# FlyCole/Dream2Real

Measured on AMD Instinct MI355X. Metric: candidate renders scored/sec (640x360), higher is better.
Workload: dtype bf16 + fp16 NeRF MLP operands (fp32 accumulate; the library's default: the reference's tiny-cuda-nn operand type, same MFMA rate; --opt mlp_f16=0 = bf16 operands)

## Files before the change

### dream2real_amd/csrc/clip.hip

```cpp
#include "d2r_internal.h"

#include <type_traits>

#include <math.h>
#include <stdio.h>
#include <stdlib.h>

#include <algorithm>
#include <deque>
#include <mutex>

typedef __bf16 bf16x8 __attribute__((ext_vector_type(8)));
typedef float f32x16 __attribute__((ext_vector_type(16)));
typedef float f32x4 __attribute__((ext_vector_type(4)));

struct ClipWeights {
    const uint16_t *w_patch;
    const float *cls, *pos;
    const float *pre_w, *pre_b;
    struct Layer {
        const float *ln1_w, *ln1_b, *ln2_w, *ln2_b;
        const uint16_t *w_qkv, *w_o, *w_fc1, *w_fc2;
        const float *b_qkv, *b_o, *b_fc1, *b_fc2;
        const uint16_t *wf_qkv = nullptr, *wf_fc1 = nullptr;
// ... 203 lines not shown
                           uint16_t *__restrict__ patches, uint32_t Kp_pad)
{
    size_t i = (size_t)blockIdx.x * blockDim.x + threadIdx.x;
    size_t total = (size_t)n * 3 * S * S;
    if (i >= total) return;
    uint32_t x = i % S, y = (i / S) % S, c = (i / ((size_t)S * S)) % 3, img = i / ((size_t)3 * S * S);
    uint32_t g = S / P;
    size_t rowi = (size_t)img * g * g + (y / P) * g + (x / P);
    patches[rowi * Kp_pad + (c * P + (y % P)) * P + (x % P)] = f2bf(pv[i]);
}


__device__ __forceinline__ size_t lo8_off(uint32_t M_pad, size_t row, uint32_t col)
{
    return ((((size_t)(col >> 6) * (M_pad >> 6)) + (row >> 6)) << 12) + ((row & 31) << 7) + (((col & 63) >> 3) << 4) + (((row >> 5) & 1) << 3) + (col & 7);
}
__device__ __forceinline__ float split8_value(uint32_t hi16, int32_t lo8) { return __uint_as_float((hi16 << 16) + (uint32_t)(lo8 << 8)); }
__device__ __forceinline__ int32_t split8_round(float x, uint32_t hi_bits )
{
    const int32_t dlt = (int32_t)__float_as_uint(x) - (int32_t)hi_bits;
    return min(dlt + 0x80, 0x7fff);
}

enum { EPI_F32 = 0, EPI_BIAS_BF16 = 1, EPI_BIAS_GELU_BF16 = 2, EPI_BIAS_RESID_F32 = 3,
       EPI_LN_BIAS_BF16 = 4, EPI_LN_BIAS_GELU_BF16 = 5, EPI_RESID_STATS_F32X = 6, EPI_RESID_STATS_BF16 = 7,
       EPI_RESID_STATS_SPLIT = 8, EPI_RESID_STATS_SPLIT8 = 9,
       EPI_F8_BIAS_BF16 = 10, EPI_F8_BIAS_GELU_Q8 = 11, EPI_F8_RESID_STATS_SPLIT8 = 12, EPI_KINDS = 13 };
#define EPI_IS_F8(E) ((E) >= EPI_F8_BIAS_BF16)
#define EPI_IS_LN(E) ((E) == EPI_LN_BIAS_BF16 || (E) == EPI_LN_BIAS_GELU_BF16)
#define EPI_IS_STATS(E) ((E) == EPI_RESID_STATS_F32X || (E) == EPI_RESID_STATS_BF16 || (E) == EPI_RESID_STATS_SPLIT || (E) == EPI_RESID_STATS_SPLIT8 || (E) == EPI_F8_RESID_STATS_SPLIT8)
#define EPI_IS_F32_LAYOUT(E) ((E) == EPI_F32 || (E) == EPI_BIAS_RESID_F32)

struct EpiAux {
    const float *cs;
    const float2 *ab;
    uint16_t *xb;
    float2 *part;
    uint16_t *xlo;
    uint32_t hm_rows;
    uint32_t a_rs, a_ks;
    const uint32_t *m_dev;
    const uint32_t *a_scale;
    float w_scale;
    uint8_t *q8;
    uint8_t *q8_scale;
};

__device__ __forceinline__ uint32_t q8_scale_byte(float amax)
{
    const int e = (int)((__float_as_uint(amax) + 0x200000u) >> 23);
    return (uint32_t)min(max(e - 8, 1), 253);
}
__device__ __forceinline__ float q8_inv_scale(uint32_t byte) { return __uint_as_float((254u - byte) << 23); }
__device__ __forceinline__ size_t q8_scale_off(uint32_t M_pad, size_t row, uint32_t group)
{
    return ((((size_t)(group >> 1) * (M_pad >> 6) + (row >> 6)) * 32 + (row & 31)) << 2) + (((row >> 5) & 1) << 1) + (group & 1u);
}
typedef float f32x2 __attribute__((ext_vector_type(2)));
__device__ __forceinline__ uint2 q8_pack8(const float (&f)[8], float inv)
{
    const f32x2 i2 = f32x2{inv, inv};
    const f32x2 q0 = f32x2{f[0], f[1]} * i2, q1 = f32x2{f[2], f[3]} * i2, q2 = f32x2{f[4], f[5]} * i2, q3 = f32x2{f[6], f[7]} * i2;
    uint32_t a = __builtin_amdgcn_cvt_pk_fp8_f32(q0[0], q0[1], 0, false);
    a = __builtin_amdgcn_cvt_pk_fp8_f32(q1[0], q1[1], a, true);
    uint32_t b = __builtin_amdgcn_cvt_pk_fp8_f32(q2[0], q2[1], 0, false);
    b = __builtin_amdgcn_cvt_pk_fp8_f32(q3[0], q3[1], b, true);
    return make_uint2(a, b);
}

#ifdef D2R_DEV
#include "clip_dev.h"
#else
#define D2R_GEMM_ABLATE 0
#define D2R_ATTN_ABLATE 0
#define D2R_F8_EXP 0
#define D2R_F8_VAR 0
#define STAMP(var)
#endif
#ifndef D2R_GEMM_LATE_DRAIN
#define D2R_GEMM_LATE_DRAIN 1
#endif
#ifndef D2R_GEMM_MFMA16
#define D2R_GEMM_MFMA16 1
#endif
#ifndef D2R_GEMM_PRIO
#define D2R_GEMM_PRIO 2
#endif
#define BM 256
#define BK 64
#define GEMM_THREADS 512

__device__ __forceinline__ uint32_t lds_off(uint32_t row, uint32_t chunk)
{
    return row * 128u + ((chunk ^ ((row >> 1) & 7u)) << 4);
}

__device__ __forceinline__ void glds16(const void *g, uint32_t lds_byte_addr)
{
    asm volatile("s_mov_b32 m0, %1\n\ts_nop 0\n\tglobal_load_lds_dwordx4 %0, off" : : "v"(g), "s"(lds_byte_addr) : "memory");
}
__device__ __forceinline__ uint32_t lds_addr(const void *p)
{
    return (uint32_t)(size_t)(__attribute__((address_space(3))) const void *)p;
}
template <int N>
__device__ __forceinline__ void wait_vmcnt()
{
    static_assert(N >= 0 && N < 64, "vmcnt is a 6-bit field");
    asm volatile("s_waitcnt vmcnt(%0)" ::"n"(N) : "memory");
}

#define EP_LD 68u
#define EP_WAVE_FLOATS (8u * EP_LD)
struct NoHook { __device__ __forceinline__ void operator()() const {} };
__device__ __forceinline__ float row16_sum(float x)
{
    x += __int_as_float(__builtin_amdgcn_update_dpp(0, __float_as_int(x), 0x128, 0xf, 0xf, false));
    x += __int_as_float(__builtin_amdgcn_update_dpp(0, __float_as_int(x), 0x124, 0xf, 0xf, false));
    x += __int_as_float(__builtin_amdgcn_update_dpp(0, __float_as_int(x), 0x122, 0xf, 0xf, false));
    x += __int_as_float(__builtin_amdgcn_update_dpp(0, __float_as_int(x), 0x121, 0xf, 0xf, false));
    return x;
}
__device__ __forceinline__ float row8_sum(float x)
{
    x += __int_as_float(__builtin_amdgcn_update_dpp(0, __float_as_int(x), 0xB1, 0xf, 0xf, false));
    x += __int_as_float(__builtin_amdgcn_update_dpp(0, __float_as_int(x), 0x4E, 0xf, 0xf, false));
    x += __int_as_float(__builtin_amdgcn_update_dpp(0, __float_as_int(x), 0x141, 0xf, 0xf, false));
    return x;
}
__device__ __forceinline__ float row8_max(float x)
{
    x = fmaxf(x, __int_as_float(__builtin_amdgcn_update_dpp(0, __float_as_int(x), 0xB1, 0xf, 0xf, false)));
    x = fmaxf(x, __int_as_float(__builtin_amdgcn_update_dpp(0, __float_as_int(x), 0x4E, 0xf, 0xf, false)));
    x = fmaxf(x, __int_as_float(__builtin_amdgcn_update_dpp(0, __float_as_int(x), 0x141, 0xf, 0xf, false)));
    return x;
}
__device__ __forceinline__ float bf_lo(uint32_t u) { return __uint_as_float(u << 16); }
__device__ __forceinline__ float bf_hi(uint32_t u) { return __uint_as_float(u & 0xffff0000u); }

template <int EPI, int MT, typename Hook = NoHook>
__device__ __forceinline__ void gemm_epilogue(f32x16 (&acc)[MT][2], float *ep, uint32_t lane,
                                              uint32_t row0, uint32_t col0, const float *__restrict__ bias,
                                              void *__restrict__ Cout, uint32_t N, const EpiAux &aux,
                                              const float2 *ab_lds, Hook hook = Hook())
{
    const uint32_t ep_addr = __builtin_amdgcn_readfirstlane(lds_addr(ep));
    auto transpose_in = [&](int i, int p8) {
        if (D2R_GEMM_ABLATE & 256) return;
        asm volatile("s_mov_b32 m0, %8\n\ts_nop 0\n\t"
                     "ds_write_addtid_b32 %0 offset:0\n\tds_write_addtid_b32 %1 offset:272\n\t"
                     "ds_write_addtid_b32 %2 offset:544\n\tds_write_addtid_b32 %3 offset:816\n\t"
                     "ds_write_addtid_b32 %4 offset:1088\n\tds_write_addtid_b32 %5 offset:1360\n\t"
                     "ds_write_addtid_b32 %6 offset:1632\n\tds_write_addtid_b32 %7 offset:1904"
                     :
                     : "v"(acc[i][0][4 * p8 + 0]), "v"(acc[i][0][4 * p8 + 1]), "v"(acc[i][0][4 * p8 + 2]), "v"(acc[i][0][4 * p8 + 3]),
                       "v"(acc[i][1][4 * p8 + 0]), "v"(acc[i][1][4 * p8 + 1]), "v"(acc[i][1][4 * p8 + 2]), "v"(acc[i][1][4 * p8 + 3]),
                       "s"(ep_addr)
                     : "memory");
    };
    static_assert(EP_LD == 68u, "the ds_write_addtid offsets above are (4 j + r) * EP_LD * 4 bytes");
    auto ep_at = [](uint32_t R, uint32_t c) -> uint32_t { return ((c >> 5) * 4u + (R & 3u)) * EP_LD + (R >> 2) * 32u + (c & 31u); };
    if (EPI_IS_F32_LAYOUT(EPI)) {
        const uint32_t c4 = (lane & 15) * 4, rl0 = lane >> 4;
        const uint32_t col = col0 + c4;
        constexpr bool RESID_F32 = EPI == EPI_BIAS_RESID_F32;
        float4 bv = make_float4(0.f, 0.f, 0.f, 0.f);
// ... 1461 lines not shown
            }
        }
    }
}

template <bool CAUSAL>
__global__ __launch_bounds__(ATTN_THREADS, 4) void k_attention(const uint16_t *__restrict__ QKV, uint16_t *__restrict__ AO, uint32_t T,
                                                              uint32_t T_pad, uint32_t d, uint32_t M_pad)
{
    constexpr uint32_t TH = ATTN_THREADS;
    extern __shared__ __attribute__((aligned(16))) uint8_t smem[];
    uint8_t *Ks = smem;
    uint16_t *Vt = (uint16_t *)(smem + (size_t)T_pad * 128);
    const uint32_t vstride = T_pad + 4;
    const uint32_t head = blockIdx.x, img = blockIdx.y;
    const uint32_t tid = threadIdx.x, lane = tid & 63, wave = tid >> 6, li = lane & 31, hi = lane >> 5;
    const size_t row_base = (size_t)img * T;
    const uint32_t ld = 64, H = d >> 6;
    const uint16_t *Qg = QKV + ((size_t)head * M_pad + row_base) * 64;
    const uint16_t *Kg = QKV + ((size_t)(H + head) * M_pad + row_base) * 64;
    const uint16_t *Vg = QKV + ((size_t)(2 * H + head) * M_pad + row_base) * 64;

    const uint32_t n_qt = (T + 31) / 32, n_kt = T_pad / 32;
    uint4 qf[4];
    {
        const uint32_t qrow0 = wave * 32 + li;
#pragma unroll
        for (int s = 0; s < 4; s++)
            qf[s] = qrow0 < T ? *(const uint4 *)(Qg + (size_t)qrow0 * ld + 16 * s + 8 * hi) : make_uint4(0, 0, 0, 0);
    }
    {
        const uint32_t ks0 = __builtin_amdgcn_readfirstlane(lds_addr(Ks));
        for (uint32_t b = __builtin_amdgcn_readfirstlane(wave); b < T_pad / 8; b += TH / 64) {
            const uint32_t row = b * 8 + (lane >> 3), src_row = row < T ? row : T - 1;
            glds16(Kg + (size_t)src_row * ld + ((lane & 7) ^ ((row >> 1) & 7u)) * 8, ks0 + b * 1024);
        }
    }
    for (uint32_t i = tid; i < (T_pad / 4) * 8; i += TH) {
        const uint32_t kb = (i >> 3) * 4, c = i & 7;
        uint4 v[4];
#pragma unroll
        for (int k = 0; k < 4; k++)
            v[k] = *(const uint4 *)(Vg + (size_t)(kb + k < T ? kb + k : T - 1) * ld + c * 8);
        const uint32_t *w0 = (const uint32_t *)&v[0], *w1 = (const uint32_t *)&v[1];
        const uint32_t *w2 = (const uint32_t *)&v[2], *w3 = (const uint32_t *)&v[3];
#pragma unroll
        for (int p = 0; p < 4; p++) {
            uint2 lo, hi2;
            lo.x = __builtin_amdgcn_perm(w1[p], w0[p], 0x05040100);
            lo.y = __builtin_amdgcn_perm(w3[p], w2[p], 0x05040100);
            hi2.x = __builtin_amdgcn_perm(w1[p], w0[p], 0x07060302);
            hi2.y = __builtin_amdgcn_perm(w3[p], w2[p], 0x07060302);
            *(uint2 *)(Vt + (size_t)(c * 8 + 2 * p) * vstride + kb) = lo;
            *(uint2 *)(Vt + (size_t)(c * 8 + 2 * p + 1) * vstride + kb) = hi2;
        }
    }
    wait_vmcnt<0>();
    __syncthreads();
    for (uint32_t qt = wave; qt < n_qt; qt += TH / 64) {
        if (qt != wave) {
            const uint32_t qrow = qt * 32 + li;
#pragma unroll
            for (int s = 0; s < 4; s++)
                qf[s] = qrow < T ? *(const uint4 *)(Qg + (size_t)qrow * ld + 16 * s + 8 * hi) : make_uint4(0, 0, 0, 0);
        }
        attn_qtile<CAUSAL>(Ks, Vt, vstride, qf, qt, T, n_kt, li, hi, AO, row_base, M_pad, head);
    }
}

#define ATTN_Q_SCALE (0.125f * 1.4426950408889634f)
#define ATS_THREADS 512
#define ATS_STAGES 5
#define ATS_SLOT 8192u
#define ATS_DEFER 8.0f
typedef short s16x4 __attribute__((ext_vector_type(4)));
typedef __attribute__((address_space(3))) const uint8_t *lds_cptr;
__device__ __forceinline__ uint2 lds_read_tr16(lds_cptr p)
{
    union { s16x4 s; uint2 u; } c;
    c.s = __builtin_amdgcn_ds_read_tr16_b64_v4i16((__attribute__((address_space(3))) s16x4 *)p);
    return c.u;
}

template <int NR>
__device__ __forceinline__ void ats_softmax(f32x16 &sacc, f32x16 &o0, f32x16 &o1, float &m_run, float &l_run, uint4 (&pb)[2])
{
#if D2R_ATTN_ABLATE & 32
    l_run += sacc[0];
    o0[0] += sacc[1];
#else
    float tmax;
    if constexpr (NR == 16) {
        float a, b;
        asm("v_max3_f32 %0, %1, %2, %3" : "=v"(a) : "v"(sacc[0]), "v"(sacc[1]), "v"(sacc[2]));
        asm("v_max3_f32 %0, %1, %2, %3" : "=v"(b) : "v"(sacc[3]), "v"(sacc[4]), "v"(sacc[5]));
        asm("v_max3_f32 %0, %1, %2, %0" : "+v"(a) : "v"(sacc[6]), "v"(sacc[7]));
        asm("v_max3_f32 %0, %1, %2, %0" : "+v"(b) : "v"(sacc[8]), "v"(sacc[9]));
        asm("v_max3_f32 %0, %1, %2, %0" : "+v"(a) : "v"(sacc[10]), "v"(sacc[11]));
        asm("v_max3_f32 %0, %1, %2, %0" : "+v"(b) : "v"(sacc[12]), "v"(sacc[13]));
        asm("v_max3_f32 %0, %1, %2, %0" : "+v"(a) : "v"(sacc[14]), "v"(sacc[15]));
        asm("v_max_f32 %0, %1, %2" : "=v"(tmax) : "v"(a), "v"(b));
    } else {
        float a;
        asm("v_max3_f32 %0, %1, %2, %3" : "=v"(a) : "v"(sacc[0]), "v"(sacc[1]), "v"(sacc[2]));
        asm("v_max_f32 %0, %1, %2" : "=v"(tmax) : "v"(a), "v"(sacc[3]));
    }
    {
        typedef unsigned u32x2 __attribute__((ext_vector_type(2)));
        const u32x2 r = __builtin_amdgcn_permlane32_swap(__float_as_uint(tmax), __float_as_uint(tmax), false, false);
        asm("v_max_f32 %0, %1, %2" : "=v"(tmax) : "v"(r[0]), "v"(r[1]));
    }
    if (__builtin_amdgcn_ballot_w64(tmax > ATS_DEFER) != 0) {
        const float dm = fmaxf(tmax, 0.f);
        const float alpha = __builtin_amdgcn_exp2f(-dm);
        l_run *= alpha;
#pragma unroll
        for (int r = 0; r < 16; r++) {
            o0[r] *= alpha;
            o1[r] *= alpha;
        }
#pragma unroll
        for (int r = 0; r < NR; r++) sacc[r] -= dm;
        m_run += dm;
    }
    if constexpr (NR == 16) {
        typedef float f32x2 __attribute__((ext_vector_type(2)));
        f32x2 pr[8];
#pragma unroll
        for (int q = 0; q < 8; q++) {
            pr[q] = f32x2{__builtin_amdgcn_exp2f(sacc[2 * q]), __builtin_amdgcn_exp2f(sacc[2 * q + 1])};
            asm volatile("" : "+v"(pr[q]));
            sacc[2 * q] = pr[q].x;
            sacc[2 * q + 1] = pr[q].y;
        }
        const f32x2 a0 = pr[0] + pr[4], a1 = pr[1] + pr[5], a2 = pr[2] + pr[6], a3 = pr[3] + pr[7];
        const f32x2 b0 = a0 + a2, b1 = a1 + a3;
        const f32x2 s2 = b0 + b1;
        l_run += s2.x + s2.y;
    } else {
#pragma unroll
        for (int r = 0; r < 4; r++) sacc[r] = __builtin_amdgcn_exp2f(sacc[r]);
        l_run += (sacc[0] + sacc[1]) + (sacc[2] + sacc[3]);
    }
#endif
    pb[0].x = pack2(sacc[0], sacc[1]);
    pb[0].y = pack2(sacc[2], sacc[3]);
    if constexpr (NR == 16) {
        pb[0].z = pack2(sacc[4], sacc[5]);
        pb[0].w = pack2(sacc[6], sacc[7]);
        pb[1] = make_uint4(pack2(sacc[8], sacc[9]), pack2(sacc[10], sacc[11]), pack2(sacc[12], sacc[13]), pack2(sacc[14], sacc[15]));
    } else {
        pb[0].z = pb[0].w = 0u;
        pb[1] = make_uint4(0u, 0u, 0u, 0u);
    }
}

template <int NW, bool Q8 = false>
__global__ __launch_bounds__(NW * 64, NW == 8 ? 4 : 1) void k_attention_s(const uint16_t *__restrict__ QKV, uint16_t *__restrict__ AO, uint32_t T,
                                                                          uint32_t d, uint32_t M_pad, uint32_t qt0, uint8_t *__restrict__ AOS = nullptr)
{
    extern __shared__ __attribute__((aligned(16))) uint8_t smem[];
    constexpr int NS = 8 / NW;
    const uint32_t head = blockIdx.x, img = blockIdx.y;
    const uint32_t tid = threadIdx.x, lane = tid & 63, wave = __builtin_amdgcn_readfirstlane(tid >> 6), li = lane & 31, hi = lane >> 5;
    const size_t row_base = (size_t)img * T;
    const uint32_t H = d >> 6;
// ... 115 lines not shown
        for (int s = 0; s < ((D2R_ATTN_ABLATE & 64) ? 0 : 2); s++) {
            if (s == 1 && short_tile) break;
            union { uint4 u; bf16x8 v; } p, va0, va1;
            p.u = pb[s];
            const uint2 a00 = lds_read_tr16(v0 + 2048u * s), a01 = lds_read_tr16(v0 + 2048u * s + 1024u);
            const uint2 a10 = lds_read_tr16(v1 + 2048u * s), a11 = lds_read_tr16(v1 + 2048u * s + 1024u);
            va0.u = make_uint4(a00.x, a00.y, a01.x, a01.y);
            va1.u = make_uint4(a10.x, a10.y, a11.x, a11.y);
            o0 = __builtin_amdgcn_mfma_f32_32x32x16_bf16(va0.v, p.v, o0, 0, 0, 0);
            o1 = __builtin_amdgcn_mfma_f32_32x32x16_bf16(va1.v, p.v, o1, 0, 0, 0);
        }
        if constexpr (!LAST) {
#pragma unroll
            for (int r = 0; r < 16; r++) sacc[r] = (D2R_ATTN_ABLATE & 128) ? __uint_as_float(ka[r & 3].x) : 0.f;
            if (!(D2R_ATTN_ABLATE & 128)) {
                typedef float f32x2 __attribute__((ext_vector_type(2)));
                f32x2 nm = {-m_run, -m_run}, pr[8];
#pragma unroll
                for (int q = 0; q < 8; q++) asm volatile("v_mov_b64 %0, %1" : "=v"(pr[q]) : "v"(nm));
#pragma unroll
                for (int q = 0; q < 8; q++) {
                    sacc[2 * q] = pr[q].x;
                    sacc[2 * q + 1] = pr[q].y;
                }
            }
#pragma unroll
            for (int s = 0; s < ((D2R_ATTN_ABLATE & 128) ? 0 : 4); s++) s_mfma(sacc, s);
        }
    };
    using std::integral_constant;
    const integral_constant<bool, false> no{};
    const integral_constant<bool, true> yes{};
    uint32_t kt = 0;
    for (; kt + ATS_STAGES - 1 < n_kt; kt++) tile(kt, integral_constant<int, ATS_STAGES - 3>{}, yes, no);
    if (n_kt - kt == 4) { tile(kt, integral_constant<int, 2>{}, no, no); kt++; }
    if (n_kt - kt == 3) { tile(kt, integral_constant<int, 1>{}, no, no); kt++; }
    if (n_kt - kt == 2) { tile(kt, integral_constant<int, 0>{}, no, no); kt++; }
    tile(kt, integral_constant<int, 0>{}, no, yes);
    wait_vmcnt<0>();
    if (!active) return;
    const float inv_l = 1.0f / half_sum(l_run);
    typedef unsigned u32x2 __attribute__((ext_vector_type(2)));
    const uint32_t lane_e = __builtin_amdgcn_mbcnt_hi(~0u, __builtin_amdgcn_mbcnt_lo(~0u, 0u));
    const uint32_t qrow_e = qt * 32 + (lane_e & 31);
    if constexpr (Q8) {
        float am = 0.f;
#pragma unroll
        for (int r = 0; r < 16; r++) am = fmaxf(am, fmaxf(fabsf(o0[r]), fabsf(o1[r])));
        am *= inv_l;
        const u32x2 ams = __builtin_amdgcn_permlane32_swap(__float_as_uint(am), __float_as_uint(am), false, false);
        const uint32_t sb = q8_scale_byte(fmaxf(__uint_as_float(ams[0]), __uint_as_float(ams[1])));
        const float sc = inv_l * q8_inv_scale(sb);
        uint8_t *dst8 = (uint8_t *)AO + (((size_t)head * M_pad + row_base + qrow_e) << 6) + 8 * (lane_e >> 5);
#pragma unroll
        for (int t = 0; t < 2; t++) {
            const f32x16 &o = t ? o1 : o0;
#pragma unroll
            for (int g = 0; g < 2; g++) {
                uint32_t a = __builtin_amdgcn_cvt_pk_fp8_f32(o[8 * g + 0] * sc, o[8 * g + 1] * sc, 0, false);
                a = __builtin_amdgcn_cvt_pk_fp8_f32(o[8 * g + 2] * sc, o[8 * g + 3] * sc, a, true);
                uint32_t b = __builtin_amdgcn_cvt_pk_fp8_f32(o[8 * g + 4] * sc, o[8 * g + 5] * sc, 0, false);
                b = __builtin_amdgcn_cvt_pk_fp8_f32(o[8 * g + 6] * sc, o[8 * g + 7] * sc, b, true);
                const u32x2 x = __builtin_amdgcn_permlane32_swap(a, b, false, false);
                if (qrow_e < T) *(uint2 *)(dst8 + 32 * t + 16 * g) = make_uint2(x[0], x[1]);
            }
        }
        if (qrow_e < T && lane_e < 32) AOS[q8_scale_off(M_pad, row_base + qrow_e, head)] = (uint8_t)sb;
        return;
    }
    uint16_t *dst = AO + ((size_t)head * M_pad + row_base + qrow_e) * 64 + 8 * (lane_e >> 5);
#pragma unroll
    for (int t = 0; t < 2; t++) {
        const f32x16 &o = t ? o1 : o0;
#pragma unroll
        for (int g = 0; g < 2; g++) {
            uint32_t a0 = pack2(o[8 * g + 0] * inv_l, o[8 * g + 1] * inv_l), a1 = pack2(o[8 * g + 2] * inv_l, o[8 * g + 3] * inv_l);
            uint32_t b0 = pack2(o[8 * g + 4] * inv_l, o[8 * g + 5] * inv_l), b1 = pack2(o[8 * g + 6] * inv_l, o[8 * g + 7] * inv_l);
            const u32x2 x = __builtin_amdgcn_permlane32_swap(a0, b0, false, false);
            const u32x2 y = __builtin_amdgcn_permlane32_swap(a1, b1, false, false);
            if (qrow_e < T) *(uint4 *)(dst + 32 * t + 16 * g) = make_uint4(x[0], y[0], x[1], y[1]);
        }
    }
}

__global__ __launch_bounds__(256) void k_attention_cls(const uint16_t *__restrict__ QKV, const uint16_t *__restrict__ Q_cls,
                                                       uint16_t *__restrict__ AO_cls, uint32_t T, uint32_t d, uint32_t M_pad,
                                                       uint32_t n_heads, uint32_t n_items)
{
    __shared__ float ps[4][1024];
    const uint32_t lane = threadIdx.x & 63, w = threadIdx.x >> 6;
    const uint32_t item = blockIdx.x * 4 + w;
    if (item >= n_items) return;
    const uint32_t img = item / n_heads, head = item - img * n_heads, H = d >> 6;
    const size_t row0 = (size_t)img * T;
    const uint16_t *Qg = Q_cls ? Q_cls + (size_t)img * d + head * 64 : QKV + ((size_t)head * M_pad + row0) * 64;
    const uint16_t *Kg = QKV + ((size_t)(H + head) * M_pad + row0) * 64;
    const uint16_t *Vg = QKV + ((size_t)(2 * H + head) * M_pad + row0) * 64;
    float q[64];
    {
        const uint4 *qp = (const uint4 *)Qg;
#pragma unroll
        for (int c = 0; c < 8; c++) {
            const uint4 v = qp[c];
            q[8 * c + 0] = bf_lo(v.x); q[8 * c + 1] = bf_hi(v.x); q[8 * c + 2] = bf_lo(v.y); q[8 * c + 3] = bf_hi(v.y);
            q[8 * c + 4] = bf_lo(v.z); q[8 * c + 5] = bf_hi(v.z); q[8 * c + 6] = bf_lo(v.w); q[8 * c + 7] = bf_hi(v.w);
        }
    }
    float mx = -INFINITY;
    for (uint32_t key = lane; key < T; key += 64) {
        const uint4 *kp = (const uint4 *)(Kg + (size_t)key * 64);
        float a = 0.f;
#pragma unroll
        for (int c = 0; c < 8; c++) {
            const uint4 v = kp[c];
            a = fmaf(q[8 * c + 0], bf_lo(v.x), a); a = fmaf(q[8 * c + 1], bf_hi(v.x), a);
            a = fmaf(q[8 * c + 2], bf_lo(v.y), a); a = fmaf(q[8 * c + 3], bf_hi(v.y), a);
            a = fmaf(q[8 * c + 4], bf_lo(v.z), a); a = fmaf(q[8 * c + 5], bf_hi(v.z), a);
            a = fmaf(q[8 * c + 6], bf_lo(v.w), a); a = fmaf(q[8 * c + 7], bf_hi(v.w), a);
        }
        ps[w][key] = a;
        mx = fmaxf(mx, a);
    }
#pragma unroll
    for (int o = 32; o > 0; o >>= 1) mx = fmaxf(mx, __shfl_xor(mx, o));
    float sum = 0.f;
    for (uint32_t key = lane; key < T; key += 64) {
        const float p = __builtin_amdgcn_exp2f(ps[w][key] - mx);
        ps[w][key] = p;
        sum += p;
    }
    sum = wave_sum(sum);
    __builtin_amdgcn_wave_barrier();
    float o = 0.f;
    for (uint32_t key = 0; key < T; key++) o = fmaf(ps[w][key], __uint_as_float((uint32_t)Vg[(size_t)key * 64 + lane] << 16), o);
    AO_cls[(size_t)img * d + head * 64 + lane] = f2bf(o / sum);
}

__global__ void k_gather_cls(const float *__restrict__ X, const uint16_t *__restrict__ Xhi, const uint16_t *__restrict__ Xlo,
                             uint32_t M_pad, uint32_t T, uint32_t d, uint32_t n, float *__restrict__ X_cls, int lo8 = 0)
{
    const uint32_t i = blockIdx.x * blockDim.x + threadIdx.x;
    if (i >= n * d) return;
    const uint32_t img = i / d, c = i - img * d;
    const size_t row = (size_t)img * T;
    float v;
    if (Xhi) {
        const size_t xo = ((size_t)(c >> 6) * M_pad + row) * 64 + (c & 63);
        v = __uint_as_float((uint32_t)Xhi[xo] << 16);
        if (Xlo && lo8) v = split8_value(Xhi[xo], ((const int8_t *)Xlo)[lo8_off(M_pad, row, c)]);
        else if (Xlo) v += __uint_as_float((uint32_t)Xlo[xo] << 16);
    } else {
        v = X[row * d + c];
    }
    X_cls[i] = v;
}

__global__ void k_gather_cls_operand(const uint16_t *__restrict__ Xhi, const float2 *__restrict__ AB, uint32_t M_pad, uint32_t T,
                                     uint32_t d, uint32_t n, uint16_t *__restrict__ Xq, float2 *__restrict__ ABq)
{
    const uint32_t i = blockIdx.x * blockDim.x + threadIdx.x, per = d / 8;
    if (i >= n * per) return;
    const uint32_t img = i / per, c = (i - img * per) * 8;
    const size_t row = (size_t)img * T;
    *(uint4 *)(Xq + (size_t)img * d + c) = *(const uint4 *)(Xhi + ((size_t)(c >> 6) * M_pad + row) * 64 + (c & 63));
    if (c == 0) ABq[img] = AB[row];
}
// ... 1081 lines not shown
```

Measured before the change: 28620.

## Rewrite CLIP attention kernel around 16x16x32 MFMA tiles with per-half-tile query handling

Adds a new default variant of the streaming attention kernel that uses 16x16x32 bf16 MFMA instead of the 32x32x16 form. Each 32-row query tile is split into two 16-row halves so a tile with only one live half skips that half's work, and the softmax reductions are rebuilt around permlane swaps for the new accumulator layout. The last key tile is masked at 16-key granularity so half-empty tails skip a V read and MFMA. It adds a second large code path, and the old ablation masks now only build with the legacy form.

After: 28620. Within noise of the previous version (-0.0%).

```diff
diff --git a/dream2real_amd/csrc/clip.hip b/dream2real_amd/csrc/clip.hip
--- a/dream2real_amd/csrc/clip.hip
+++ b/dream2real_amd/csrc/clip.hip
@@ -309,6 +309,12 @@
 #endif
 #ifndef D2R_GEMM_MFMA16
 #define D2R_GEMM_MFMA16 1
+#endif
+#ifndef D2R_ATTN_MFMA16
+#define D2R_ATTN_MFMA16 1
+#endif
+#if D2R_ATTN_MFMA16 && D2R_ATTN_ABLATE
+#error "the D2R_ATTN_ABLATE masks are wired into the 32x32x16 form of k_attention_s only: build them with -DD2R_ATTN_MFMA16=0"
 #endif
 #ifndef D2R_GEMM_PRIO
 #define D2R_GEMM_PRIO 2
@@ -1936,6 +1942,7 @@
     return c.u;
 }
 
+#if !D2R_ATTN_MFMA16
 template <int NR>
 __device__ __forceinline__ void ats_softmax(f32x16 &sacc, f32x16 &o0, f32x16 &o1, float &m_run, float &l_run, uint4 (&pb)[2])
 {
@@ -2217,6 +2224,331 @@
         }
     }
 }
+#else
+template <int NQ>
+__device__ __forceinline__ float ats_qmax(float (&t)[2])
+{
+    typedef unsigned u32x2 __attribute__((ext_vector_type(2)));
+    float x;
+    u32x2 r = __builtin_amdgcn_permlane32_swap(__float_as_uint(t[0]), __float_as_uint(t[NQ - 1]), false, false);
+    asm("v_max_f32 %0, %1, %2" : "=v"(x) : "v"(r[0]), "v"(r[1]));
+    r = __builtin_amdgcn_permlane16_swap(__float_as_uint(x), __float_as_uint(x), false, false);
+    asm("v_max_f32 %0, %1, %2" : "=v"(x) : "v"(r[0]), "v"(r[1]));
+    if constexpr (NQ == 2) {
+        r = __builtin_amdgcn_permlane32_swap(__float_as_uint(x), __float_as_uint(x), false, false);
+        t[0] = __uint_as_float(r[0]);
+        t[1] = __uint_as_float(r[1]);
+    } else {
+        t[0] = x;
+    }
+    return x;
+}
+template <int NQ>
+__device__ __forceinline__ void ats_qsum(float (&t)[2])
+{
+    typedef unsigned u32x2 __attribute__((ext_vector_type(2)));
+    u32x2 r = __builtin_amdgcn_permlane32_swap(__float_as_uint(t[0]), __float_as_uint(t[NQ - 1]), false, false);
+    float x = __uint_as_float(r[0]) + __uint_as_float(r[1]);
+    r = __builtin_amdgcn_permlane16_swap(__float_as_uint(x), __float_as_uint(x), false, false);
+    x = __uint_as_float(r[0]) + __uint_as_float(r[1]);
+    if constexpr (NQ == 2) {
+        r = __builtin_amdgcn_permlane32_swap(__float_as_uint(x), __float_as_uint(x), false, false);
+        t[0] = __uint_as_float(r[0]);
+        t[1] = __uint_as_float(r[1]);
+    } else {
+        t[0] = x;
+    }
+}
+
+typedef float f32x2 __attribute__((ext_vector_type(2)));
+typedef unsigned ats_u32x4 __attribute__((ext_vector_type(4)));
+template <int NK, int NQ>
+__device__ __forceinline__ void ats_softmax(f32x4 (&s)[2][2], f32x4 (&o)[4][2], f32x2 (&nm_run)[2], f32x2 (&l_run)[2], ats_u32x4 (&pb)[2])
+{
+    float t[2];
+#pragma unroll
+    for (int qb = 0; qb < NQ; qb++) {
+        float a;
+        asm("v_max3_f32 %0, %1, %2, %3" : "=v"(a) : "v"(s[0][qb][0]), "v"(s[0][qb][1]), "v"(s[0][qb][2]));
+        if constexpr (NK == 2) {
+            asm("v_max3_f32 %0, %1, %2, %0" : "+v"(a) : "v"(s[0][qb][3]), "v"(s[1][qb][0]));
+            asm("v_max3_f32 %0, %1, %2, %0" : "+v"(a) : "v"(s[1][qb][1]), "v"(s[1][qb][2]));
+            asm("v_max_f32 %0, %1, %2" : "=v"(t[qb]) : "v"(a), "v"(s[1][qb][3]));
+        } else {
+            asm("v_max_f32 %0, %1, %2" : "=v"(t[qb]) : "v"(a), "v"(s[0][qb][3]));
+        }
+    }
+    const float vote = ats_qmax<NQ>(t);
+    if (__builtin_amdgcn_ballot_w64(vote > ATS_DEFER) != 0) {
+#pragma unroll
+        for (int qb = 0; qb < NQ; qb++) {
+            const float dm = fmaxf(t[qb], 0.f);
+            const float alpha = __builtin_amdgcn_exp2f(-dm);
+            l_run[qb] *= alpha;
+#pragma unroll
+            for (int db = 0; db < 4; db++) o[db][qb] *= alpha;
+#pragma unroll
+            for (int kb = 0; kb < NK; kb++) s[kb][qb] -= dm;
+            nm_run[qb] -= dm;
+        }
+    }
+#pragma unroll
+    for (int qb = 0; qb < NQ; qb++) {
+        f32x2 pr[2 * NK];
+#pragma unroll
+        for (int kb = 0; kb < NK; kb++)
+#pragma unroll
+            for (int h = 0; h < 2; h++) {
+                f32x2 &p = pr[2 * kb + h];
+                p = f32x2{__builtin_amdgcn_exp2f(s[kb][qb][2 * h]), __builtin_amdgcn_exp2f(s[kb][qb][2 * h + 1])};
+                asm volatile("" : "+v"(p));
+                s[kb][qb][2 * h] = p.x;
+                s[kb][qb][2 * h + 1] = p.y;
+            }
+        auto pk_add = [](f32x2 a, f32x2 b) {
+            f32x2 r;
+            asm("v_pk_add_f32 %0, %1, %2" : "=v"(r) : "v"(a), "v"(b));
+            return r;
+        };
+        if constexpr (NK == 2) l_run[qb] = pk_add(l_run[qb], pk_add(pk_add(pr[0], pr[2]), pk_add(pr[1], pr[3])));
+        else l_run[qb] = pk_add(l_run[qb], pk_add(pr[0], pr[1]));
+        pb[qb][0] = pack2(s[0][qb][0], s[0][qb][1]);
+        pb[qb][1] = pack2(s[0][qb][2], s[0][qb][3]);
+        if constexpr (NK == 2) {
+            pb[qb][2] = pack2(s[1][qb][0], s[1][qb][1]);
+            pb[qb][3] = pack2(s[1][qb][2], s[1][qb][3]);
+        } else {
+            pb[qb][2] = pb[qb][3] = 0u;
+        }
+    }
+}
+
+template <int NW, bool Q8 = false>
+__global__ __launch_bounds__(NW * 64, NW == 8 ? 4 : 1) void k_attention_s(const uint16_t *__restrict__ QKV, uint16_t *__restrict__ AO, uint32_t T,
+                                                                          uint32_t d, uint32_t M_pad, uint32_t qt0, uint8_t *__restrict__ AOS = nullptr)
+{
+    extern __shared__ __attribute__((aligned(16))) uint8_t smem[];
+    constexpr int NS = 8 / NW;
+    const uint32_t head = blockIdx.x, img = blockIdx.y;
+    const uint32_t tid = threadIdx.x, lane = tid & 63, wave = __builtin_amdgcn_readfirstlane(tid >> 6), l16 = lane & 15, g = lane >> 4;
+    const size_t row_base = (size_t)img * T;
+    const uint32_t H = d >> 6;
+    const uint32_t n_kt = (T + 31) / 32;
+    const uint32_t qt = qt0 + blockIdx.z * NW + wave;
+    const bool active = __builtin_amdgcn_readfirstlane(qt < n_kt ? 1u : 0u) != 0u;
+    const bool one_qb = __builtin_amdgcn_readfirstlane(qt * 32 + 16 >= T ? 1u : 0u) != 0u;
+    const uint16_t *Qg = QKV + ((size_t)head * M_pad + row_base) * 64;
+    const uint16_t *src_k = QKV + ((size_t)(H + head) * M_pad + row_base) * 64, *src_v = QKV + ((size_t)(2 * H + head) * M_pad + row_base) * 64;
+    const uint32_t smem0 = __builtin_amdgcn_readfirstlane(lds_addr(smem));
+    uint32_t slot_req = 0, slot_k = 0, slot_v = 0;
+    auto advance = [](uint32_t &slot) { slot = slot + ATS_SLOT == ATS_STAGES * ATS_SLOT ? 0u : slot + ATS_SLOT; };
+    uint32_t src_off[NS], dst_off[NS], r_loc[NS];
+    bool is_v[NS];
+#pragma unroll
+    for (int j = 0; j < NS; j++) {
+        const uint32_t c = wave + (uint32_t)j * NW;
+        is_v[j] = c >= 4;
+        r_loc[j] = (c & 3) * 8 + (is_v[j] ? (lane >> 1) & 7u : lane >> 3);
+        src_off[j] = (is_v[j] ? 2 * (lane >> 4) + (lane & 1) : (lane & 7) ^ ((r_loc[j] >> 1) & 7u)) * 8;
+        dst_off[j] = (is_v[j] ? 4096u : 0u) + (c & 3) * 1024u;
+    }
+    auto request = [&](uint32_t kt) {
+#pragma unroll
+        for (int j = 0; j < NS; j++) {
+            const uint32_t row = kt * 32 + r_loc[j];
+            glds16((is_v[j] ? src_v : src_k) + (size_t)(row < T ? row : T - 1) * 64 + src_off[j], smem0 + slot_req + dst_off[j]);
+        }
+        advance(slot_req);
+    };
+    ats_u32x4 qv[4];
+    {
+        const uint32_t qrow = qt * 32 + l16;
+        const uint32_t qr0 = active && qrow < T ? qrow : T - 1, qr1 = active && qrow + 16 < T ? qrow + 16 : T - 1;
+        const uint16_t *qp0 = Qg + (size_t)qr0 * 64 + 8 * g, *qp1 = Qg + (size_t)qr1 * 64 + 8 * g;
+        asm volatile("global_load_dwordx4 %0, %4, off\n\tglobal_load_dwordx4 %1, %4, off offset:64\n\t"
+                     "global_load_dwordx4 %2, %5, off\n\tglobal_load_dwordx4 %3, %5, off offset:64"
+                     : "=&v"(qv[0]), "=&v"(qv[1]), "=&v"(qv[2]), "=&v"(qv[3]) : "v"(qp0), "v"(qp1) : "memory");
+    }
+    static_assert(ATS_STAGES == 5, "the waits below are written for a five-slot ring");
+#pragma unroll
+    for (uint32_t c = 0; c < ATS_STAGES - 1; c++) request(c);
+    asm volatile("s_waitcnt vmcnt(%4)" : "+v"(qv[0]), "+v"(qv[1]), "+v"(qv[2]), "+v"(qv[3]) : "n"(4 * NS) : "memory");
+    wait_vmcnt<3 * NS>();
+    __syncthreads();
+
+    uint32_t koff[2];
+#pragma unroll
+    for (int kk = 0; kk < 2; kk++) koff[kk] = lds_off(l16, 4 * kk + g);
+    const uint32_t vrow = 4 * g + (l16 >> 2);
+    const uint32_t voff = 4096u + (vrow >> 3) * 1024u + (vrow & 7u) * 32u + (l16 & 3u) * 8u;
+    const uint32_t n_last = T - (n_kt - 1) * 32;
+
+    f32x4 o[4][2], s[2][2];
+    f32x2 nm_run[2] = {f32x2{0.f, 0.f}, f32x2{0.f, 0.f}};
+    f32x2 l_run[2] = {f32x2{0.f, 0.f}, f32x2{0.f, 0.f}};
+    ats_u32x4 ka[2][2];
+    auto read_k = [&]() {
+#pragma unroll
+        for (int kb = 0; kb < 2; kb++)
+#pragma unroll
+            for (int kk = 0; kk < 2; kk++) ka[kb][kk] = *(const __attribute__((address_space(3))) ats_u32x4 *)((lds_cptr)(size_t)(smem0 + slot_k + koff[kk]) + 2048u * kb);
+        advance(slot_k);
+    };
+    auto mfma = [](ats_u32x4 a, ats_u32x4 b, f32x4 &acc) {
+        acc = __builtin_amdgcn_mfma_f32_16x16x32_bf16(__builtin_bit_cast(bf16x8, a), __builtin_bit_cast(bf16x8, b), acc, 0, 0, 0);
+    };
+    using std::integral_constant;
+    const integral_constant<bool, false> no{};
+    const integral_constant<bool, true> yes{};
+    auto run = [&](auto nq_tag) {
+        constexpr int NQ = decltype(nq_tag)::value;
+        auto s_mfma = [&]() {
+#pragma unroll
+            for (int kk = 0; kk < 2; kk++)
+#pragma unroll
+                for (int kb = 0; kb < 2; kb++)
+#pragma unroll
+                    for (int qb = 0; qb < NQ; qb++) mfma(ka[kb][kk], qv[2 * qb + kk], s[kb][qb]);
+        };
+#pragma unroll
+        for (int db = 0; db < 4; db++)
+#pragma unroll
+            for (int qb = 0; qb < 2; qb++) o[db][qb] = f32x4{0.f, 0.f, 0.f, 0.f};
+        read_k();
+        if (active) {
+#pragma unroll
+            for (int kb = 0; kb < 2; kb++)
+#pragma unroll
+                for (int qb = 0; qb < 2; qb++) s[kb][qb] = f32x4{0.f, 0.f, 0.f, 0.f};
+            s_mfma();
+            float t[2] = {0.f, 0.f};
+#pragma unroll
+            for (int qb = 0; qb < NQ; qb++) {
+                t[qb] = s[0][qb][0];
+#pragma unroll
+                for (int r = 1; r < 8; r++) t[qb] = fmaxf(t[qb], s[r >> 2][qb][r & 3]);
+            }
+            ats_qmax<NQ>(t);
+#pragma unroll
+            for (int qb = 0; qb < NQ; qb++) {
+                nm_run[qb] = f32x2{-t[qb], -t[qb]};
+#pragma unroll
+                for (int kb = 0; kb < 2; kb++) s[kb][qb] -= t[qb];
+            }
+        }
+        auto tile = [&](uint32_t kt, auto wait_tag, auto req_tag, auto last_tag) {
+            constexpr int WAIT = decltype(wait_tag)::value;
+            constexpr bool LAST = decltype(last_tag)::value, REQ = decltype(req_tag)::value;
+            if constexpr (!LAST) {
+                wait_vmcnt<WAIT * NS>();
+                __syncthreads();
+                if constexpr (REQ) request(kt + ATS_STAGES - 1);
+                read_k();
+            }
+            const lds_cptr vp = (lds_cptr)(size_t)(smem0 + slot_v + voff);
+            advance(slot_v);
+            if (!active) return;
+            ats_u32x4 pb[2];
+            auto pv = [&](auto full_tag) {
+#pragma unroll
+                for (int db = 0; db < 4; db++) {
+                    const uint2 a0 = lds_read_tr16(vp + 256u * db);
+                    const uint2 a1 = decltype(full_tag)::value ? lds_read_tr16(vp + 256u * db + 2048u) : make_uint2(0u, 0u);
+#pragma unroll
+                    for (int qb = 0; qb < NQ; qb++) mfma(ats_u32x4{a0.x, a0.y, a1.x, a1.y}, pb[qb], o[db][qb]);
+                }
+            };
+            if (LAST && n_last <= 16) {
+#pragma unroll
+                for (int qb = 0; qb < NQ; qb++)
+#pragma unroll
+                    for (int r = 0; r < 4; r++) s[0][qb][r] = 4 * g + (uint32_t)r < n_last ? s[0][qb][r] : -INFINITY;
+                ats_softmax<1, NQ>(s, o, nm_run, l_run, pb);
+                pv(no);
+            } else {
+                if (LAST && n_last < 32) {
+#pragma unroll
+                    for (int qb = 0; qb < NQ; qb++)
+#pragma unroll
+                        for (int r = 0; r < 4; r++) s[1][qb][r] = 16 + 4 * g + (uint32_t)r < n_last ? s[1][qb][r] : -INFINITY;
+                }
+                ats_softmax<2, NQ>(s, o, nm_run, l_run, pb);
+                pv(yes);
+            }
+            if constexpr (!LAST) {
+#pragma unroll
+                for (int qb = 0; qb < NQ; qb++) {
+                    const f32x2 nm = nm_run[qb];
+#pragma unroll
+                    for (int kb = 0; kb < 2; kb++) {
+                        f32x2 lo, hi;
+                        asm volatile("v_mov_b64 %0, %1" : "=v"(lo) : "v"(nm));
+                        asm volatile("v_mov_b64 %0, %1" : "=v"(hi) : "v"(nm));
+                        s[kb][qb] = f32x4{lo.x, lo.y, hi.x, hi.y};
+                    }
+                }
+                s_mfma();
+            }
+        };
+        uint32_t kt = 0;
+        for (; kt + ATS_STAGES - 1 < n_kt; kt++) tile(kt, integral_constant<int, ATS_STAGES - 3>{}, yes, no);
+        if (n_kt - kt == 4) { tile(kt, integral_constant<int, 2>{}, no, no); kt++; }
+        if (n_kt - kt == 3) { tile(kt, integral_constant<int, 1>{}, no, no); kt++; }
+        if (n_kt - kt == 2) { tile(kt, integral_constant<int, 0>{}, no, no); kt++; }
+        tile(kt, integral_constant<int, 0>{}, no, yes);
+        wait_vmcnt<0>();
+        if (!active) return;
+        float inv_l[2];
+#pragma unroll
+        for (int qb = 0; qb < 2; qb++) inv_l[qb] = l_run[qb].x + l_run[qb].y;
+        ats_qsum<NQ>(inv_l);
+#pragma unroll
+        for (int qb = 0; qb < NQ; qb++) inv_l[qb] = 1.0f / inv_l[qb];
+        typedef unsigned u32x2 __attribute__((ext_vector_type(2)));
+        const uint32_t lane_e = __builtin_amdgcn_mbcnt_hi(~0u, __builtin_amdgcn_mbcnt_lo(~0u, 0u));
+        const uint32_t ge = lane_e >> 4, dim_e = 16 * (ge & 1) + 8 * (ge >> 1);
+#pragma unroll
+        for (int qb = 0; qb < NQ; qb++) {
+            const uint32_t qrow_e = qt * 32 + 16 * qb + (lane_e & 15);
+            if constexpr (Q8) {
+                float am[2] = {0.f, 0.f};
+#pragma unroll
+                for (int db = 0; db < 4; db++)
+#pragma unroll
+                    for (int r = 0; r < 4; r++) am[0] = fmaxf(am[0], fabsf(o[db][qb][r]));
+                am[0] *= inv_l[qb];
+                ats_qmax<1>(am);
+                const uint32_t sb = q8_scale_byte(am[0]);
+                const float sc = inv_l[qb] * q8_inv_scale(sb);
+                uint8_t *dst8 = (uint8_t *)AO + (((size_t)head * M_pad + row_base + qrow_e) << 6) + dim_e;
+#pragma unroll
+                for (int dp = 0; dp < 2; dp++) {
+                    const f32x4 &oa = o[2 * dp][qb], &ob = o[2 * dp + 1][qb];
+                    uint32_t a = __builtin_amdgcn_cvt_pk_fp8_f32(oa[0] * sc, oa[1] * sc, 0, false);
+                    a = __builtin_amdgcn_cvt_pk_fp8_f32(oa[2] * sc, oa[3] * sc, a, true);
+                    uint32_t b = __builtin_amdgcn_cvt_pk_fp8_f32(ob[0] * sc, ob[1] * sc, 0, false);
+                    b = __builtin_amdgcn_cvt_pk_fp8_f32(ob[2] * sc, ob[3] * sc, b, true);
+                    const u32x2 x = __builtin_amdgcn_permlane16_swap(a, b, false, false);
+                    if (qrow_e < T) *(uint2 *)(dst8 + 32 * dp) = make_uint2(x[0], x[1]);
+                }
+                if (qrow_e < T && lane_e < 16) AOS[q8_scale_off(M_pad, row_base + qrow_e, head)] = (uint8_t)sb;
+            } else {
+                uint16_t *dst = AO + ((size_t)head * M_pad + row_base + qrow_e) * 64 + dim_e;
+                const float il = inv_l[qb];
+#pragma unroll
+                for (int dp = 0; dp < 2; dp++) {
+                    const f32x4 &oa = o[2 * dp][qb], &ob = o[2 * dp + 1][qb];
+                    const u32x2 x = __builtin_amdgcn_permlane16_swap(pack2(oa[0] * il, oa[1] * il), pack2(ob[0] * il, ob[1] * il), false, false);
+                    const u32x2 y = __builtin_amdgcn_permlane16_swap(pack2(oa[2] * il, oa[3] * il), pack2(ob[2] * il, ob[3] * il), false, false);
+                    if (qrow_e < T) *(uint4 *)(dst + 32 * dp) = make_uint4(x[0], y[0], x[1], y[1]);
+                }
+            }
+        }
+    };
+    if (active && one_qb) run(integral_constant<int, 1>{});
+    else run(integral_constant<int, 2>{});
+}
+#endif
 
 __global__ __launch_bounds__(256) void k_attention_cls(const uint16_t *__restrict__ QKV, const uint16_t *__restrict__ Q_cls,
                                                        uint16_t *__restrict__ AO_cls, uint32_t T, uint32_t d, uint32_t M_pad,
```
